# mttga/purejaxql

Hardware: NVIDIA H100
Metric: MinAtar-Breakout env steps/sec @4096 envs x128 seeds (higher is better)
Workload: dtype f32

## Files before the change

include/pqn_b200.h:

```cpp
#ifndef PQN_B200_H
#define PQN_B200_H

#include <stdint.h>

#ifdef __cplusplus
extern "C" {
#endif

#define PQN_OK 0
#define PQN_E_INVALID (-1)
#define PQN_E_CUDA (-2)
#define PQN_E_UNSUPPORTED (-3)

#define PQN_ENV_BREAKOUT 0
#define PQN_ENV_ASTERIX 1
#define PQN_ENV_SPACE_INVADERS 2
#define PQN_ENV_FREEWAY 3
#define PQN_ENV_SEAQUEST 4
#define PQN_ENV_CARTPOLE 16
#define PQN_ENV_ACROBOT 17
#define PQN_ENV_MOUNTAIN_CAR 18
#define PQN_ENV_MEMORY_CHAIN 32
#define PQN_ENV_CATCH 33
#define PQN_ENV_DEEP_SEA 34
// ... 99 lines not shown

int pqn_net_layout(const pqn_net_desc_t* desc_host, pqn_net_layout_t* out_host);
int pqn_net_dense_layer(const pqn_net_desc_t* desc_host, int32_t layer, int64_t* offsets_host);
int64_t pqn_net_stats_floats(const pqn_net_desc_t* desc_host);
int64_t pqn_net_workspace_bytes(const pqn_net_desc_t* desc_host, int32_t S, int64_t rows);

int pqn_net_init(const pqn_net_desc_t* desc_host, const uint32_t* keys, float* params, int32_t S, void* stream);

int pqn_qnet_forward(const pqn_net_desc_t* desc_host, const float* params, const float* batch_stats, const void* obs,
                     const int32_t* gather, int64_t obs_rows_per_seed, float* q, int32_t S, int64_t rows,
                     void* workspace, void* stream);

int pqn_qnet_loss_grad(const pqn_net_desc_t* desc_host, const float* params, float* batch_stats, const void* obs,
                       const int32_t* gather, int64_t obs_rows_per_seed, const int32_t* action,
                       const float* target, int64_t tr_rows_per_seed, float* grads, float* loss_sum,
                       float* qsa_sum, float* bn_sums, int32_t S, int64_t rows, void* workspace, void* stream);

int pqn_rnn_step(const pqn_net_desc_t* desc_host, const float* params, float* hs, const float* obs,
                 int64_t obs_rows_per_seed, const uint8_t* last_done, const int32_t* last_action, float* q, int32_t S,
                 int32_t E, void* workspace, void* stream);
int pqn_rnn_loss_grad(const pqn_net_desc_t* desc_host, const float* params, const float* hs0, const float* obs,
                      const uint8_t* last_done, const int32_t* last_action, const int32_t* action, const float* reward,
                      const uint8_t* done, float* grads, float* loss_sum, float* qsa_sum, int32_t S, int32_t T, int32_t B,
                      float gamma, float lambda, void* workspace, void* stream);
int pqn_rnn_step_stats(const pqn_net_desc_t* desc_host, const float* params, const float* batch_stats, float* hs,
                       const float* obs, int64_t obs_rows_per_seed, const uint8_t* last_done, const int32_t* last_action,
                       float* q, int32_t S, int32_t E, void* workspace, void* stream);
int pqn_rnn_loss_grad_stats(const pqn_net_desc_t* desc_host, const float* params, float* batch_stats, const float* hs0,
                            const float* obs, const uint8_t* last_done, const int32_t* last_action,
                            const int32_t* action, const float* reward, const uint8_t* done, float* grads,
                            float* loss_sum, float* qsa_sum, int32_t S, int32_t T, int32_t B, float gamma, float lambda,
                            void* workspace, void* stream);

int pqn_radam_clip_step(float* params, const float* grads, float* mu, float* nu, const float* sched,
                        int32_t* step_counter, float* gnorm_scratch , int32_t S, int64_t P,
                        float max_norm, float b1, float b2, float eps, void* stream);

int pqn_bn_stats_update(float* batch_stats, float* bn_sums, int32_t S, int32_t F, int64_t stats_seed_stride,
                        float count, float momentum, void* stream);

int pqn_set_tensor_core_path(int on);
int pqn_set_conv_mma_path(int on);

int pqn_tc_split_lo(const float* x, float* lo, int64_t n, void* stream);
int pqn_tc_gemm_test(const float* a, const float* a_lo, const float* b, const float* b_lo, float* d, int32_t S,
                     int32_t M, int32_t N, int32_t K, int a_mn, int b_mn, int split3, void* stream);

int pqn_tc_split16(const float* x, void* hi, void* lo, int64_t n, float scale, void* stream);
int pqn_tc_gemm16_test(const void* a_hi, const void* a_lo, const void* b_hi, const void* b_lo, float* d, int32_t S,
                       int32_t M, int32_t N, int32_t K, int a_mn, int b_mn, float out_scale, void* stream);
int pqn_tc_dgrad16_test(const void* a_hi, const void* a_lo, const void* b_hi, const void* b_lo, const float* mask,
                        const uint32_t* relu_bits, float* d, int32_t S, int32_t M, int32_t N, int32_t K, int epi,
                        float out_scale, void* stream);

#ifdef __cplusplus
}
#endif
#endif
```

purejaxql_b200/_lib.py:

```python
from __future__ import annotations

import ctypes
import os
from ctypes import POINTER, Structure, c_char_p, c_double, c_float, c_int, c_int32, c_int64, c_longlong, c_void_p

HERE = os.path.dirname(os.path.abspath(__file__))
LIB_PATH = os.path.join(HERE, "libpqn_b200.so")


class EnvInfo(Structure):
    _fields_ = [("state_words", c_int32), ("obs_dim", c_int32), ("obs_shape", c_int32 * 3),
                ("num_actions", c_int32), ("max_steps", c_int32), ("binary_obs", c_int32),
                ("packed_obs_words", c_int32)]


class EnvParams(Structure):
    _fields_ = [("max_steps", c_int32), ("memory_length", c_int32)]


class NetDesc(Structure):
    _fields_ = [("kind", c_int32), ("in_c", c_int32), ("hidden", c_int32), ("layers", c_int32),
                ("num_actions", c_int32), ("norm_type", c_int32), ("norm_input", c_int32)]


# ... 25 lines not shown
    "pqn_threefry2x32": (c_int, [c_void_p, c_void_p, c_void_p, c_int64, c_void_p]),
    "pqn_rng_bits": (c_int, [c_void_p, c_int64, c_int64, c_void_p, c_int, c_void_p]),
    "pqn_random_normal": (c_int, [c_void_p, c_void_p, c_int64, c_int, c_void_p]),
    "pqn_normal_from_bits": (c_int, [c_void_p, c_void_p, c_int64, c_void_p]),
    "pqn_set_permutation_bucket_log2": (c_int, [c_int]),
    "pqn_permutation_workspace_bytes": (c_int64, [c_int64, c_int]),
    "pqn_permutation": (c_int, [c_void_p, c_int64, c_int, c_int, c_void_p, c_int64, c_void_p, c_void_p]),
    "pqn_env_reset": (c_int, [c_int, c_void_p, c_void_p, c_void_p, c_int64, c_int, c_int, c_void_p]),
    "pqn_env_reset_params": (c_int, [c_int, c_void_p, c_void_p, c_void_p, c_int64, POINTER(EnvParams), c_int, c_void_p]),
    "pqn_env_step": (c_int, [c_int, c_void_p, c_void_p, c_void_p, c_void_p, c_void_p, c_void_p, c_void_p,
                             c_void_p, c_void_p, c_void_p, c_int64, c_int, c_int, c_void_p]),
    "pqn_env_obs_packed": (c_int, [c_int, c_void_p, c_void_p, c_int64, c_void_p]),
    "pqn_env_obs": (c_int, [c_int, c_void_p, c_void_p, c_int64, c_void_p]),
    "pqn_eps_greedy": (c_int, [c_void_p, c_void_p, c_void_p, c_void_p, c_int64, c_int32, c_int, c_void_p]),
    "pqn_rollout_act_step": (c_int, [c_int, c_void_p, c_void_p, c_void_p, c_void_p, c_void_p, c_int64, c_void_p,
                                     c_void_p, c_void_p, c_void_p, c_int64, c_void_p, c_int, c_int32, c_int32,
                                     c_int32, c_int32, c_int, c_float, c_int, c_void_p]),
    "pqn_rollout_keys": (c_int, [c_void_p, c_void_p, c_int32, c_int32, c_int, c_void_p]),
    "pqn_qlambda": (c_int, [c_void_p, c_void_p, c_void_p, c_void_p, c_void_p, c_int32, c_int32, c_int32, c_int32,
                            c_float, c_float, c_void_p]),
    "pqn_net_layout": (c_int, [POINTER(NetDesc), POINTER(NetLayout)]),
    "pqn_net_dense_layer": (c_int, [POINTER(NetDesc), c_int32, POINTER(c_int64)]),
    "pqn_net_stats_floats": (c_int64, [POINTER(NetDesc)]),
    "pqn_net_workspace_bytes": (c_int64, [POINTER(NetDesc), c_int32, c_int64]),
    "pqn_net_init": (c_int, [POINTER(NetDesc), c_void_p, c_void_p, c_int32, c_void_p]),
    "pqn_qnet_forward": (c_int, [POINTER(NetDesc), c_void_p, c_void_p, c_void_p, c_void_p, c_int64, c_void_p, c_int32,
                                 c_int64, c_void_p, c_void_p]),
    "pqn_qnet_loss_grad": (c_int, [POINTER(NetDesc), c_void_p, c_void_p, c_void_p, c_void_p, c_int64, c_void_p,
                                   c_void_p, c_int64, c_void_p, c_void_p, c_void_p, c_void_p, c_int32, c_int64,
                                   c_void_p, c_void_p]),
    "pqn_rnn_step": (c_int, [POINTER(NetDesc), c_void_p, c_void_p, c_void_p, c_int64, c_void_p, c_void_p, c_void_p,
                             c_int32, c_int32, c_void_p, c_void_p]),
    "pqn_rnn_loss_grad": (c_int, [POINTER(NetDesc), c_void_p, c_void_p, c_void_p, c_void_p, c_void_p, c_void_p, c_void_p,
                                  c_void_p, c_void_p, c_void_p, c_void_p, c_int32, c_int32, c_int32, c_float, c_float,
                                  c_void_p, c_void_p]),
    "pqn_rnn_step_stats": (c_int, [POINTER(NetDesc), c_void_p, c_void_p, c_void_p, c_void_p, c_int64, c_void_p, c_void_p,
                                   c_void_p, c_int32, c_int32, c_void_p, c_void_p]),
    "pqn_rnn_loss_grad_stats": (c_int, [POINTER(NetDesc), c_void_p, c_void_p, c_void_p, c_void_p, c_void_p, c_void_p,
                                        c_void_p, c_void_p, c_void_p, c_void_p, c_void_p, c_void_p, c_int32, c_int32,
                                        c_int32, c_float, c_float, c_void_p, c_void_p]),
    "pqn_radam_clip_step": (c_int, [c_void_p, c_void_p, c_void_p, c_void_p, c_void_p, c_void_p, c_void_p, c_int32,
                                    c_int64, c_float, c_float, c_float, c_float, c_void_p]),
    "pqn_bn_stats_update": (c_int, [c_void_p, c_void_p, c_int32, c_int32, c_int64, c_float, c_float, c_void_p]),
    "pqn_set_tensor_core_path": (c_int, [c_int]),
    "pqn_set_conv_mma_path": (c_int, [c_int]),
    "pqn_tc_split_lo": (c_int, [c_void_p, c_void_p, c_int64, c_void_p]),
    "pqn_tc_split16": (c_int, [c_void_p, c_void_p, c_void_p, c_int64, c_float, c_void_p]),
    "pqn_tc_gemm_test": (c_int, [c_void_p, c_void_p, c_void_p, c_void_p, c_void_p, c_int32, c_int32, c_int32,
                                 c_int32, c_int, c_int, c_int, c_void_p]),
    "pqn_tc_gemm16_test": (c_int, [c_void_p, c_void_p, c_void_p, c_void_p, c_void_p, c_int32, c_int32, c_int32,
                                   c_int32, c_int, c_int, c_float, c_void_p]),
    "pqn_tc_dgrad16_test": (c_int, [c_void_p, c_void_p, c_void_p, c_void_p, c_void_p, c_void_p, c_void_p, c_int32,
                                    c_int32, c_int32, c_int32, c_int, c_float, c_void_p]),
}

EXPORTS = tuple(_SIGS)
_lib = None


def lib():
    global _lib
    if _lib is None:
        if not os.path.exists(LIB_PATH):
            raise PqnError(
                f"{LIB_PATH} is not built. Run `python -m purejaxql_b200.build` (needs nvcc). "
                "purejaxql_b200 has no CPU fallback.")
        l = ctypes.CDLL(LIB_PATH)
        for name, (res, args) in _SIGS.items():
            fn = getattr(l, name)
            fn.restype = res
            fn.argtypes = args
        _lib = l
    return _lib


def check(rc: int, what: str = ""):
    if rc != 0:
        msg = lib().pqn_last_error().decode("utf-8", "replace")
        raise PqnError(f"{what or 'libpqn_b200'} failed (rc={rc}): {msg}")


def p(t):
    if t is None:
        return None
    if not t.is_cuda:
        raise PqnError("libpqn_b200 takes CUDA tensors only (no CPU fallback); got a CPU tensor")
    if not t.is_contiguous():
        raise PqnError("libpqn_b200 takes contiguous tensors")
    return c_void_p(t.data_ptr())


def raw(t):
    if t is None:
        return None
    if not t.is_cuda:
        raise PqnError("libpqn_b200 takes CUDA tensors only (no CPU fallback); got a CPU tensor")
    return c_void_p(t.data_ptr())


def stream_ptr():
    import torch
    return c_void_p(torch.cuda.current_stream().cuda_stream)


def profile_read(reset=True):
    l = lib()
# ... 6 lines not shown
```

purejaxql_b200/csrc/pqn_tc.cu:

```cuda
#include <cuda.h>
#include <cuda_runtime.h>
#include <stdint.h>

#include "../../include/pqn_b200.h"
#include "api_common.h"
#include "tc_common.cuh"

namespace pqn {
namespace tc {

constexpr int STG_LD = 36;

__device__ __forceinline__ void store_chunk_coalesced(float* stage, const float (&vals)[32], int lane, float* dst,
                                                      int64_t ld, int m_base, int M) {
#pragma unroll
  for (int j = 0; j < 8; ++j)
    *reinterpret_cast<float4*>(stage + lane * STG_LD + 4 * j) =
        make_float4(vals[4 * j], vals[4 * j + 1], vals[4 * j + 2], vals[4 * j + 3]);
  __syncwarp();
  const int r_in = lane >> 3, c4 = lane & 7;
#pragma unroll
  for (int it = 0; it < 8; ++it) {
    const int r = it * 4 + r_in;
    if (m_base + r < M)
// ... 46 lines not shown
  const float rstd = 1.0f / sqrtf(var + 1e-6f);
  const int64_t grow = (int64_t)seed * ep.rows + m;
  if constexpr (EPI == EPI_LN_TRAIN) {
    float* hbase = ep.H + ((int64_t)seed * ep.rows + m_base) * 128;
    float* xbase = ep.XHAT + ((int64_t)seed * ep.rows + m_base) * 128;
#pragma unroll
    for (int c = 0; c < 4; ++c) {
      float xh[32], h[32];
#pragma unroll
      for (int j4 = 0; j4 < 8; ++j4) {
        const float4 s4 = *reinterpret_cast<const float4*>(sp + SP_SC + c * 32 + 4 * j4);
        const float4 b4 = *reinterpret_cast<const float4*>(sp + SP_BI + c * 32 + 4 * j4);
        const float ss[4] = {s4.x, s4.y, s4.z, s4.w}, bb[4] = {b4.x, b4.y, b4.z, b4.w};
#pragma unroll
        for (int e = 0; e < 4; ++e) {
          const int j = 4 * j4 + e;
          xh[j] = (acc[c * 32 + j] - mean) * rstd;
          h[j] = fmaxf(xh[j] * ss[e] + bb[e], 0.f);
        }
      }
      store_chunk_coalesced(stage, h, lane, hbase + c * 32, 128, m_base, M);
      store_chunk_coalesced(stage, xh, lane, xbase + c * 32, 128, m_base, M);
    }
    if (row_ok) ep.RSTD[grow] = rstd;
  } else {
    float q[PQN_TC_MAX_A];
#pragma unroll
    for (int a = 0; a < PQN_TC_MAX_A; ++a) q[a] = 0.f;
#pragma unroll
    for (int j4 = 0; j4 < 32; ++j4) {
      const float4 s4 = *reinterpret_cast<const float4*>(sp + SP_SC + 4 * j4);
      const float4 b4 = *reinterpret_cast<const float4*>(sp + SP_BI + 4 * j4);
      float h[4];
      h[0] = fmaxf((acc[4 * j4 + 0] - mean) * rstd * s4.x + b4.x, 0.f);
      h[1] = fmaxf((acc[4 * j4 + 1] - mean) * rstd * s4.y + b4.y, 0.f);
      h[2] = fmaxf((acc[4 * j4 + 2] - mean) * rstd * s4.z + b4.z, 0.f);
      h[3] = fmaxf((acc[4 * j4 + 3] - mean) * rstd * s4.w + b4.w, 0.f);
#pragma unroll
      for (int a = 0; a < PQN_TC_MAX_A; ++a)
        if (a < ep.A) {
          const float4 w4 = *reinterpret_cast<const float4*>(sp + SP_HW + a * 128 + 4 * j4);
          q[a] = fmaf(h[0], w4.x, q[a]); q[a] = fmaf(h[1], w4.y, q[a]);
          q[a] = fmaf(h[2], w4.z, q[a]); q[a] = fmaf(h[3], w4.w, q[a]);
        }
    }
    if (row_ok) {
#pragma unroll
      for (int a = 0; a < PQN_TC_MAX_A; ++a)
        if (a < ep.A) ep.Q[grow * ep.A + a] = q[a] + sp[SP_HB + a];
    }
  }
}

template <int MN>
__device__ __forceinline__ float lds_tf32(const uint8_t* tile, int r, int k) {
  const int off = MN ? ((r >> 5) * 4096 + k * 128 + ((((r & 31) >> 2) ^ (k & 7)) << 4) + ((r & 3) << 2))
                     : (r * 128 + (((k >> 2) ^ (r & 7)) << 4) + ((k & 3) << 2));
  return *reinterpret_cast<const float*>(tile + off);
}
__device__ __forceinline__ uint32_t tf32_trunc_bits(float x) { return __float_as_uint(x) & 0xFFFFE000u; }
__device__ __forceinline__ void mma_tf32_16x8x8(float (&d)[4], const uint32_t (&a)[4], uint32_t b0, uint32_t b1) {
  asm volatile(
      "mma.sync.aligned.m16n8k8.row.col.f32.tf32.tf32.f32 {%0,%1,%2,%3}, {%4,%5,%6,%7}, {%8,%9}, {%0,%1,%2,%3};"
      : "+f"(d[0]), "+f"(d[1]), "+f"(d[2]), "+f"(d[3])
      : "r"(a[0]), "r"(a[1]), "r"(a[2]), "r"(a[3]), "r"(b0), "r"(b1));
}

template <int A_MN, int B_MN>
__device__ __forceinline__ void tf32_tile(const uint8_t* smem_al, float* tile_s, uint64_t* full, uint64_t* empty,
                                          int& stage, uint32_t& phase, int kbn, int split3, float osc, int warp,
                                          int lane) {
  const int g = lane >> 2, tq = lane & 3;
  const int wr = (warp & 3) * 32, wc = (warp >> 2) * 64;
  float mainacc[2][8][4], corr[2][8][4];
#pragma unroll
  for (int mi = 0; mi < 2; ++mi)
#pragma unroll
    for (int ni = 0; ni < 8; ++ni)
#pragma unroll
      for (int e = 0; e < 4; ++e) { mainacc[mi][ni][e] = 0.f; corr[mi][ni][e] = 0.f; }
  for (int kb = 0; kb < kbn; ++kb) {
    mbar_wait(&full[stage], phase);
    const uint8_t* sb = smem_al + stage * TC_STAGE_BYTES;
    if (kb % TC_PROMOTE == 0) {
#pragma unroll
      for (int mi = 0; mi < 2; ++mi)
#pragma unroll
        for (int ni = 0; ni < 8; ++ni)
#pragma unroll
          for (int e = 0; e < 4; ++e) mainacc[mi][ni][e] = 0.f;
    }
#pragma unroll
    for (int ks = 0; ks < TC_BK / 8; ++ks) {
      const int k = ks * 8 + tq;
      uint32_t ahi[2][4], alo[2][4];
#pragma unroll
      for (int mi = 0; mi < 2; ++mi) {
        const int r0 = wr + mi * 16 + g;
        const int rr[4] = {r0, r0 + 8, r0, r0 + 8}, kk[4] = {k, k, k + 4, k + 4};
#pragma unroll
        for (int e = 0; e < 4; ++e) {
          const float x = lds_tf32<A_MN>(sb + TC_A_HI, rr[e], kk[e]);
          ahi[mi][e] = tf32_trunc_bits(x);
          const float lo = split3 == 1 ? lds_tf32<A_MN>(sb + TC_A_LO, rr[e], kk[e]) : x - __uint_as_float(ahi[mi][e]);
          alo[mi][e] = tf32_trunc_bits(lo);
        }
      }
#pragma unroll
      for (int ni = 0; ni < 8; ++ni) {
        const int n = wc + ni * 8 + g;
        const uint32_t bh0 = tf32_trunc_bits(lds_tf32<B_MN>(sb + TC_B_HI, n, k));
        const uint32_t bh1 = tf32_trunc_bits(lds_tf32<B_MN>(sb + TC_B_HI, n, k + 4));
        if (split3) {
          const uint32_t bl0 = tf32_trunc_bits(lds_tf32<B_MN>(sb + TC_B_LO, n, k));
          const uint32_t bl1 = tf32_trunc_bits(lds_tf32<B_MN>(sb + TC_B_LO, n, k + 4));
#pragma unroll
          for (int mi = 0; mi < 2; ++mi) {
            mma_tf32_16x8x8(corr[mi][ni], alo[mi], bh0, bh1);
            mma_tf32_16x8x8(corr[mi][ni], ahi[mi], bl0, bl1);
          }
        }
#pragma unroll
        for (int mi = 0; mi < 2; ++mi) mma_tf32_16x8x8(mainacc[mi][ni], ahi[mi], bh0, bh1);
      }
    }
    __syncwarp();
    if (lane == 0) mbar_arrive(&empty[stage]);
    if (++stage == TC_STAGES) { stage = 0; phase ^= 1u; }
    if ((kb + 1) % TC_PROMOTE == 0 || kb == kbn - 1) {
      const bool first = kb < TC_PROMOTE;
#pragma unroll
      for (int mi = 0; mi < 2; ++mi)
#pragma unroll
        for (int ni = 0; ni < 8; ++ni)
#pragma unroll
          for (int h = 0; h < 2; ++h) {
            float2* p = reinterpret_cast<float2*>(tile_s + (wr + mi * 16 + g + 8 * h) * TC_ACC_LD + wc + ni * 8 + 2 * tq);
            const float2 v = make_float2(mainacc[mi][ni][2 * h], mainacc[mi][ni][2 * h + 1]);
            if (first) *p = v;
            else { const float2 o = *p; *p = make_float2(o.x + v.x, o.y + v.y); }
          }
    }
  }
#pragma unroll
  for (int mi = 0; mi < 2; ++mi)
#pragma unroll
    for (int ni = 0; ni < 8; ++ni)
#pragma unroll
      for (int h = 0; h < 2; ++h) {
        float2* p = reinterpret_cast<float2*>(tile_s + (wr + mi * 16 + g + 8 * h) * TC_ACC_LD + wc + ni * 8 + 2 * tq);
        float2 o = kbn > 0 ? *p : make_float2(0.f, 0.f);
        o.x += corr[mi][ni][2 * h];
        o.y += corr[mi][ni][2 * h + 1];
        *p = make_float2(o.x * osc, o.y * osc);
      }
}

template <int EPI, bool F16>
__host__ __device__ constexpr bool tma_store_epilogue() { return F16 && (EPI == EPI_RELU_MASK || EPI == EPI_RELU_BITS); }

__device__ __forceinline__ void wg_bar_sync(int wg) { asm volatile("bar.sync %0, 128;" ::"r"(3 + wg) : "memory"); }

template <int A_MN, int B_MN, int EPI, bool F16 = true>
__global__ void __launch_bounds__(TC_THREADS, 1)
    tc_gemm_kernel(const __grid_constant__ CUtensorMap tm_a_hi, const __grid_constant__ CUtensorMap tm_a_lo,
                   const __grid_constant__ CUtensorMap tm_b_hi, const __grid_constant__ CUtensorMap tm_b_lo,
                   const __grid_constant__ CUtensorMap tm_out, const GemmShape gs, const EpiParams ep) {
  constexpr bool TMA_EPI = tma_store_epilogue<EPI, F16>();
  extern __shared__ __align__(1024) uint8_t smem_raw[];
  const uint32_t smem_base = (smem_u32(smem_raw) + 1023u) & ~1023u;
  uint8_t* smem_al = smem_raw + (smem_base - smem_u32(smem_raw));
  float* tile_s = reinterpret_cast<float*>(smem_al + TC_STAGES * TC_STAGE_BYTES);
  float* sp_all = tile_s + 128 * TC_ACC_LD;
  uint64_t* full = reinterpret_cast<uint64_t*>(sp_all + TC_SP_FLOATS);
  uint64_t* empty = full + TC_STAGES;

  const int warp = threadIdx.x >> 5, lane = threadIdx.x & 31;

  if (warp == 8 && lane == 0) {
    prefetch_tmap(&tm_a_hi); prefetch_tmap(&tm_a_lo); prefetch_tmap(&tm_b_hi); prefetch_tmap(&tm_b_lo);
    if (TMA_EPI) prefetch_tmap(&tm_out);
    for (int i = 0; i < TC_STAGES; ++i) { mbar_init(&full[i], 1); mbar_init(&empty[i], TC_CONSUMERS / 32); }
    fence_barrier_init();
  }
  __syncthreads();

  const int ksplit = gs.k_split > 1 ? gs.k_split : 1;
  const int kb_per = (gs.k_blocks + ksplit - 1) / ksplit;
  const int tiles_per_seed = gs.m_tiles * gs.n_tiles * ksplit;
  const int num_tiles = tiles_per_seed * gs.S;
  auto decode = [&](int tile, int& seed, int& m0, int& n0, int& kb0, int& kbn) {
    seed = tile / tiles_per_seed;
    const int rem = tile - seed * tiles_per_seed;
    const int ks = rem % ksplit, mn = rem / ksplit;
    m0 = (mn / gs.n_tiles) * 128; n0 = (mn % gs.n_tiles) * 128;
    kb0 = ks * kb_per;
    kbn = min(kb_per, gs.k_blocks - kb0);
    if (kbn < 0) kbn = 0;
    return ks;
  };

  constexpr int BKE = F16 ? TC_BK16 : TC_BK;
  constexpr int MNB = F16 ? 2 : 4;
  constexpr int MNB_ELEMS = F16 ? 64 : 32, MNB_BYTES = F16 ? 8192 : 4096;
  const bool a_lo_tma = F16 || gs.split3 == 1, b_lo_tma = F16 || gs.split3 != 0;
  if (warp == 8) {
    if (lane == 0) {
      int stage = 0;
      uint32_t phase = 0;
      for (int tile = blockIdx.x; tile < num_tiles; tile += gridDim.x) {
        int seed, m0, n0, kb0, kbn;
        decode(tile, seed, m0, n0, kb0, kbn);
        for (int kb = kb0; kb < kb0 + kbn; ++kb) {
          mbar_wait(&empty[stage], phase ^ 1u);
          const uint32_t sb = smem_base + stage * TC_STAGE_BYTES;
          mbar_expect_tx(&full[stage], (2 + (a_lo_tma ? 1 : 0) + (b_lo_tma ? 1 : 0)) * TC_TILE_BYTES);
          const int k0 = kb * BKE;
          if (A_MN) {
#pragma unroll
            for (int j = 0; j < MNB; ++j) {
              tma_load_3d(sb + TC_A_HI + j * MNB_BYTES, &tm_a_hi, &full[stage], m0 + MNB_ELEMS * j, k0, seed);
              if (a_lo_tma) tma_load_3d(sb + TC_A_LO + j * MNB_BYTES, &tm_a_lo, &full[stage], m0 + MNB_ELEMS * j, k0, seed);
            }
          } else {
            tma_load_3d(sb + TC_A_HI, &tm_a_hi, &full[stage], k0, m0, seed);
            if (a_lo_tma) tma_load_3d(sb + TC_A_LO, &tm_a_lo, &full[stage], k0, m0, seed);
          }
          if (B_MN) {
#pragma unroll
            for (int j = 0; j < MNB; ++j) {
              tma_load_3d(sb + TC_B_HI + j * MNB_BYTES, &tm_b_hi, &full[stage], n0 + MNB_ELEMS * j, k0, seed);
              if (b_lo_tma) tma_load_3d(sb + TC_B_LO + j * MNB_BYTES, &tm_b_lo, &full[stage], n0 + MNB_ELEMS * j, k0, seed);
            }
          } else {
            tma_load_3d(sb + TC_B_HI, &tm_b_hi, &full[stage], k0, n0, seed);
            if (b_lo_tma) tma_load_3d(sb + TC_B_LO, &tm_b_lo, &full[stage], k0, n0, seed);
          }
          if (++stage == TC_STAGES) { stage = 0; phase ^= 1u; }
        }
      }
    }
    return;
  }

  const int t = threadIdx.x;
  const int wg = t >> 7;
  const uint32_t a_off = wg * 8192;
  const int fr = 64 * wg + 16 * ((t & 127) >> 5) + (lane >> 2), fc = 2 * (lane & 3);
  const int et = t & 127;
  uint8_t* out_stage = reinterpret_cast<uint8_t*>(tile_s) + wg * TC_OUT_STAGE_WG;
  int stage = 0;
  uint32_t phase = 0;
  for (int tile = blockIdx.x; tile < num_tiles; tile += gridDim.x) {
    int seed, m0, n0, kb0, kbn;
    const int ks_idx = decode(tile, seed, m0, n0, kb0, kbn);
    uint32_t rbits[2][4];
    if constexpr (TMA_EPI) {
      if constexpr (EPI == EPI_RELU_BITS) {
#pragma unroll
        for (int h = 0; h < 2; ++h) {
          const int m = m0 + fr + 8 * h;
          const uint4 w = m < gs.M ? __ldg(reinterpret_cast<const uint4*>(
                                         ep.relu_bits + ((int64_t)seed * ep.rows + m) * (ep.ld_out >> 5) + (n0 >> 5)))
                                   : make_uint4(0u, 0u, 0u, 0u);
          rbits[h][0] = w.x; rbits[h][1] = w.y; rbits[h][2] = w.z; rbits[h][3] = w.w;
        }
      } else {
        const int m = m0 + 64 * wg + (et >> 1);
        const float* p = ep.mask + (int64_t)seed * ep.out_seed_stride + (int64_t)m * ep.ld_out + n0 + 64 * (et & 1);
        if (m < gs.M) {
          asm volatile("prefetch.global.L2 [%0];" ::"l"(p));
          asm volatile("prefetch.global.L2 [%0];" ::"l"(p + 32));
        }
      }
      if (kbn > TC_PROMOTE) {
        if (et == 0) bulk_wait_read_all();
        wg_bar_sync(wg);
      }
    } else {
      consumer_bar_sync();
    }
    if constexpr (!F16) {
      tf32_tile<A_MN, B_MN>(smem_al, tile_s, full, empty, stage, phase, kbn, gs.split3,
                            ep.out_scale != 0.f ? ep.out_scale : 1.0f, warp, lane);
    } else {
    float mainacc[64], corr[64];
#pragma unroll
    for (int i = 0; i < 64; ++i) { mainacc[i] = 0.f; corr[i] = 0.f; }
    for (int kb = 0; kb < kbn; ++kb) {
      mbar_wait(&full[stage], phase);
      const uint32_t sb = smem_base + stage * TC_STAGE_BYTES;
      const uint32_t first_corr = kb == 0 ? 0u : 1u, first_main = kb % TC_PROMOTE == 0 ? 0u : 1u;
      fence_operands(mainacc); fence_operands(corr);
      wgmma_fence();
#pragma unroll
      for (int ks = 0; ks < 4; ++ks) {
        const uint64_t a_hi = make_gdesc16<A_MN>(sb + TC_A_HI + a_off, ks), a_lo = make_gdesc16<A_MN>(sb + TC_A_LO + a_off, ks);
        const uint64_t b_hi = make_gdesc16<B_MN>(sb + TC_B_HI, ks), b_lo = make_gdesc16<B_MN>(sb + TC_B_LO, ks);
        wgmma_f16_m64n128<A_MN, B_MN>(corr, a_lo, b_hi, ks == 0 ? first_corr : 1u);
        wgmma_f16_m64n128<A_MN, B_MN>(corr, a_hi, b_lo, 1u);
        wgmma_f16_m64n128<A_MN, B_MN>(mainacc, a_hi, b_hi, ks == 0 ? first_main : 1u);
      }
      wgmma_commit();
      wgmma_wait<0>();
      fence_operands(mainacc); fence_operands(corr);
      __syncwarp();
      if (lane == 0) mbar_arrive(&empty[stage]);
      if (++stage == TC_STAGES) { stage = 0; phase ^= 1u; }
      const bool promote = TMA_EPI ? (kb + 1) % TC_PROMOTE == 0 && kb != kbn - 1
                                   : (kb + 1) % TC_PROMOTE == 0 || kb == kbn - 1;
      if (promote) {
        const bool first = kb < TC_PROMOTE;
#pragma unroll
        for (int j = 0; j < 16; ++j)
#pragma unroll
          for (int h = 0; h < 2; ++h) {
            float2* p = reinterpret_cast<float2*>(tile_s + (fr + 8 * h) * TC_ACC_LD + 8 * j + fc);
            const float2 v = make_float2(mainacc[4 * j + 2 * h], mainacc[4 * j + 2 * h + 1]);
            if (first) *p = v;
            else { const float2 o = *p; *p = make_float2(o.x + v.x, o.y + v.y); }
          }
      }
    }
    if constexpr (TMA_EPI) {
      const float osc = ep.out_scale != 0.f ? ep.out_scale : 1.0f;
      const float* mrow = ep.mask + (int64_t)seed * ep.out_seed_stride + n0;
#pragma unroll
      for (int j = 0; j < 16; ++j)
#pragma unroll
        for (int h = 0; h < 2; ++h) {
          const int i = 4 * j + 2 * h;
          float2 o = make_float2(mainacc[i], mainacc[i + 1]);
          if (kbn > TC_PROMOTE) {
            const float2 p = *reinterpret_cast<const float2*>(tile_s + (fr + 8 * h) * TC_ACC_LD + 8 * j + fc);
            o = make_float2(p.x + o.x, p.y + o.y);
          }
          mainacc[i] = fmaf(corr[i], TC_LO_INV, o.x) * osc;
          mainacc[i + 1] = fmaf(corr[i + 1], TC_LO_INV, o.y) * osc;
        }
#pragma unroll
      for (int j = 0; j < 16; ++j)
#pragma unroll
        for (int h = 0; h < 2; ++h) {
          float& x = mainacc[4 * j + 2 * h];
          float& y = mainacc[4 * j + 2 * h + 1];
          if constexpr (EPI == EPI_RELU_BITS) {
            const uint32_t b = rbits[h][j >> 2] >> (8 * (j & 3) + fc);
            x = (b & 1u) ? x : 0.f; y = (b & 2u) ? y : 0.f;
          } else {
            const int m = m0 + fr + 8 * h;
            if (m < gs.M) {
              const float2 mk = *reinterpret_cast<const float2*>(mrow + (int64_t)m * ep.ld_out + 8 * j + fc);
              x = mk.x > 0.f ? x : 0.f; y = mk.y > 0.f ? y : 0.f;
            }
          }
        }
      if (et == 0) bulk_wait_read_all();
      wg_bar_sync(wg);
      const int rl = fr - 64 * wg;
#pragma unroll
      for (int j = 0; j < 16; ++j)
#pragma unroll
        for (int h = 0; h < 2; ++h) {
          const int chunk = 2 * (j & 3) + (fc >> 2);
          const int off = (j >> 2) * TC_OUT_BOX_BYTES + (rl + 8 * h) * 128 + ((chunk ^ (lane >> 2)) << 4) + (fc & 3) * 4;
          *reinterpret_cast<float2*>(out_stage + off) = make_float2(mainacc[4 * j + 2 * h], mainacc[4 * j + 2 * h + 1]);
        }
      fence_proxy_async_smem();
      wg_bar_sync(wg);
      if (et == 0) {
#pragma unroll
        for (int b = 0; b < 4; ++b)
          tma_store_3d(&tm_out, smem_u32(out_stage + b * TC_OUT_BOX_BYTES), n0 + 32 * b, m0 + 64 * wg, seed);
        bulk_commit();
      }
      continue;
    }
    {
      const float osc = ep.out_scale != 0.f ? ep.out_scale : 1.0f;
#pragma unroll
      for (int j = 0; j < 16; ++j)
#pragma unroll
        for (int h = 0; h < 2; ++h) {
          float2* p = reinterpret_cast<float2*>(tile_s + (fr + 8 * h) * TC_ACC_LD + 8 * j + fc);
          float2 o = kbn > 0 ? *p : make_float2(0.f, 0.f);
          if (kbn > 0) {
            o.x = fmaf(corr[4 * j + 2 * h], TC_LO_INV, o.x);
            o.y = fmaf(corr[4 * j + 2 * h + 1], TC_LO_INV, o.y);
          }
          *p = make_float2(o.x * osc, o.y * osc);
        }
    }
// ... 181 lines not shown

int pqn_tc_split16(const float* x, void* hi, void* lo, int64_t n, float scale, void* stream) {
  if (!x || !hi || !lo || n < 0 || (n & 3)) return set_error(PQN_E_INVALID, "pqn_tc_split16: bad argument (n %% 4 == 0)");
  if (n == 0) return PQN_OK;
  {
    LaunchScope _ls(K_TC_SPLIT, (cudaStream_t)stream);
    split16_kernel<<<(unsigned)((n / 4 + 255) / 256), 256, 0, (cudaStream_t)stream>>>(x, (__half*)hi, (__half*)lo, n / 4,
                                                                                       scale);
  }
  return check_launch("pqn_tc_split16");
}

int pqn_tc_gemm16_test(const void* a_hi, const void* a_lo, const void* b_hi, const void* b_lo, float* d, int32_t S,
                       int32_t M, int32_t N, int32_t K, int a_mn, int b_mn, float out_scale, void* stream) {
  if (!a_hi || !a_lo || !b_hi || !b_lo || !d || S <= 0 || M <= 0 || N <= 0 || K <= 0 || (N % 128) || (K % 8) || (M % 8))
    return set_error(PQN_E_INVALID, "pqn_tc_gemm16_test: bad argument");
  CUtensorMap t[4];
  int rc;
  const void* ap[2] = {a_hi, a_lo};
  const void* bp[2] = {b_hi, b_lo};
  for (int i = 0; i < 2; ++i) {
    if (a_mn) { if ((rc = make_tmap16(&t[i], ap[i], M, K, S, M, (uint64_t)M * K, 64))) return rc; }
    else { if ((rc = make_tmap16(&t[i], ap[i], K, M, S, K, (uint64_t)M * K, 128))) return rc; }
    if (b_mn) { if ((rc = make_tmap16(&t[2 + i], bp[i], N, K, S, N, (uint64_t)N * K, 64))) return rc; }
    else { if ((rc = make_tmap16(&t[2 + i], bp[i], K, N, S, K, (uint64_t)N * K, 128))) return rc; }
  }
  GemmShape gs = {};
  gs.S = S; gs.M = M; gs.m_tiles = (M + 127) / 128; gs.n_tiles = N / 128; gs.k_blocks = (K + TC_BK16 - 1) / TC_BK16;
  EpiParams ep = {};
  ep.out = d; ep.ld_out = N; ep.out_seed_stride = (int64_t)M * N; ep.out_scale = out_scale;
  return launch_gemm16(a_mn, b_mn, EPI_STORE, t, gs, ep, (cudaStream_t)stream);
}

int pqn_tc_dgrad16_test(const void* a_hi, const void* a_lo, const void* b_hi, const void* b_lo, const float* mask,
                        const uint32_t* relu_bits, float* d, int32_t S, int32_t M, int32_t N, int32_t K, int epi,
                        float out_scale, void* stream) {
  if (!a_hi || !a_lo || !b_hi || !b_lo || !d || S <= 0 || M <= 0 || N <= 0 || K <= 0 || (N % 128) || (K % 8) ||
      (M % 8) || !(epi == EPI_STORE || epi == EPI_RELU_MASK || epi == EPI_RELU_BITS) ||
      (epi == EPI_RELU_MASK && !mask) || (epi == EPI_RELU_BITS && !relu_bits))
    return set_error(PQN_E_INVALID, "pqn_tc_dgrad16_test: bad argument");
  CUtensorMap t[4];
  int rc;
  const void* p[4] = {a_hi, a_lo, b_hi, b_lo};
  for (int i = 0; i < 2; ++i) {
    if ((rc = make_tmap16(&t[i], p[i], K, M, S, K, (uint64_t)M * K, 128))) return rc;
    if ((rc = make_tmap16(&t[2 + i], p[2 + i], K, N, S, K, (uint64_t)N * K, 128))) return rc;
  }
  GemmShape gs = {};
  gs.S = S; gs.M = M; gs.m_tiles = (M + 127) / 128; gs.n_tiles = N / 128; gs.k_blocks = (K + TC_BK16 - 1) / TC_BK16;
  EpiParams ep = {};
  ep.out = d; ep.mask = mask; ep.relu_bits = relu_bits; ep.rows = M;
  ep.ld_out = N; ep.out_seed_stride = (int64_t)M * N; ep.out_scale = out_scale;
  return launch_gemm16(0, 0, epi, t, gs, ep, (cudaStream_t)stream);
}

int pqn_tc_gemm_test(const float* a, const float* a_lo, const float* b, const float* b_lo, float* d, int32_t S,
                     int32_t M, int32_t N, int32_t K, int a_mn, int b_mn, int split3, void* stream) {
  if (!a || !b || !d || S <= 0 || M <= 0 || N <= 0 || K <= 0 || (N % 128) || split3 < 0 || split3 > 2 ||
      (split3 && !b_lo) || (split3 == 1 && !a_lo))
    return set_error(PQN_E_INVALID, "pqn_tc_gemm_test: bad argument");
  CUtensorMap t[4];
  int rc;
  const float* al = split3 == 1 ? a_lo : a;
  const float* bl = split3 ? b_lo : b;
  const float* ap[2] = {a, al};
  const float* bp[2] = {b, bl};
  for (int i = 0; i < 2; ++i) {
    if (a_mn) { if ((rc = make_tmap(&t[i], ap[i], M, K, S, M, (uint64_t)M * K, 32))) return rc; }
    else { if ((rc = make_tmap(&t[i], ap[i], K, M, S, K, (uint64_t)M * K, 128))) return rc; }
    if (b_mn) { if ((rc = make_tmap(&t[2 + i], bp[i], N, K, S, N, (uint64_t)N * K, 32))) return rc; }
    else { if ((rc = make_tmap(&t[2 + i], bp[i], K, N, S, K, (uint64_t)N * K, 128))) return rc; }
  }
  GemmShape gs = {};
  gs.S = S; gs.M = M; gs.m_tiles = (M + 127) / 128; gs.n_tiles = N / 128; gs.k_blocks = (K + TC_BK - 1) / TC_BK;
  gs.split3 = split3;
  EpiParams ep = {};
  ep.out = d; ep.ld_out = N; ep.out_seed_stride = (int64_t)M * N;
  return launch_gemm(a_mn, b_mn, EPI_STORE, t, gs, ep, (cudaStream_t)stream);
}

}
```

purejaxql_b200/csrc/tc_common.cuh:

```cuda
#pragma once
#include <cuda.h>
#include <cuda_fp16.h>
#include <stdint.h>

namespace pqn {
namespace tc {

constexpr int TC_CONSUMERS = 256;
constexpr int TC_THREADS = TC_CONSUMERS + 32;
constexpr int TC_BK16 = 64;
constexpr int TC_BK = 32;
constexpr int TC_STAGES = 2;
constexpr int TC_PROMOTE = 4;
constexpr int TC_TILE_BYTES = 128 * TC_BK16 * 2;
constexpr float TC_LO_SCALE = 2048.0f, TC_LO_INV = 1.0f / 2048.0f;
constexpr int TC_A_HI = 0, TC_A_LO = TC_TILE_BYTES, TC_B_HI = 2 * TC_TILE_BYTES, TC_B_LO = 3 * TC_TILE_BYTES;
constexpr int TC_STAGE_BYTES = 4 * TC_TILE_BYTES;
constexpr int TC_ACC_LD = 132;
constexpr int TC_SP_FLOATS = 384 + 8 * 128 + 8;
constexpr int TC_SMEM_BYTES = TC_STAGES * TC_STAGE_BYTES + 128 * TC_ACC_LD * 4 + TC_SP_FLOATS * 4 + 256  +
                              1024 ;
constexpr int TC_OUT_BOX_BYTES = 64 * 32 * 4;
constexpr int TC_OUT_STAGE_WG = 34 * 1024;
static_assert(TC_OUT_STAGE_WG >= 64 * TC_ACC_LD * 4 && TC_OUT_STAGE_WG + 4 * TC_OUT_BOX_BYTES <= 128 * TC_ACC_LD * 4,
              "each warpgroup's output staging lies within its own 64 rows of the fp32 tile, 1024-byte aligned");
#define PQN_TC_MAX_A 8

enum Epilogue : int { EPI_STORE = 0, EPI_LN_TRAIN = 1, EPI_LN_HEAD = 2, EPI_RELU_MASK = 3, EPI_RELU_BITS = 4 };

struct GemmShape {
  int S;
  int M;
  int m_tiles, n_tiles, k_blocks;
  int split3;
  int k_split;
};

struct EpiParams {
  int64_t split_stride;
  float out_scale;
  float* out;
  const float* mask;
  const uint32_t* relu_bits;
  int64_t ld_out, out_seed_stride;
  const float* params;
  int64_t P, off_b, off_scale, off_bias, off_hw, off_hb;
  int A, rows;
  float *H, *XHAT, *RSTD, *Q;
};

__device__ __forceinline__ uint32_t smem_u32(const void* p) { return (uint32_t)__cvta_generic_to_shared(p); }

__device__ __forceinline__ float tf32_lo(float x) {
  const float hi = __uint_as_float(__float_as_uint(x) & 0xFFFFE000u);
  return x - hi;
}

__device__ __forceinline__ void mbar_init(uint64_t* bar, int count) {
  asm volatile("mbarrier.init.shared::cta.b64 [%0], %1;" ::"r"(smem_u32(bar)), "r"(count) : "memory");
}
__device__ __forceinline__ void fence_barrier_init() { asm volatile("fence.mbarrier_init.release.cluster;" ::: "memory"); }
__device__ __forceinline__ void mbar_expect_tx(uint64_t* bar, uint32_t bytes) {
  asm volatile("mbarrier.arrive.expect_tx.shared::cta.b64 _, [%0], %1;" ::"r"(smem_u32(bar)), "r"(bytes) : "memory");
}
__device__ __forceinline__ void mbar_arrive(uint64_t* bar) {
  asm volatile("mbarrier.arrive.shared::cta.b64 _, [%0];" ::"r"(smem_u32(bar)) : "memory");
}
__device__ __forceinline__ void mbar_wait(uint64_t* bar, uint32_t parity) {
  const uint32_t addr = smem_u32(bar);
  uint32_t ok;
  do {
    asm volatile(
        "{\n\t.reg .pred p;\n\t"
        "mbarrier.try_wait.parity.shared::cta.b64 p, [%1], %2;\n\t"
        "selp.u32 %0, 1, 0, p;\n\t}"
        : "=r"(ok)
        : "r"(addr), "r"(parity)
        : "memory");
  } while (!ok);
}

__device__ __forceinline__ void prefetch_tmap(const CUtensorMap* tm) {
  asm volatile("prefetch.tensormap [%0];" ::"l"(reinterpret_cast<uint64_t>(tm)) : "memory");
}
__device__ __forceinline__ void tma_load_3d(uint32_t smem_dst, const CUtensorMap* tm, uint64_t* bar, int c0, int c1, int c2) {
  asm volatile(
      "cp.async.bulk.tensor.3d.shared::cluster.global.mbarrier::complete_tx::bytes [%0], [%1, {%3, %4, %5}], [%2];"
      ::"r"(smem_dst), "l"(reinterpret_cast<uint64_t>(tm)), "r"(smem_u32(bar)), "r"(c0), "r"(c1), "r"(c2)
      : "memory");
}
__device__ __forceinline__ void tma_store_3d(const CUtensorMap* tm, uint32_t smem_src, int c0, int c1, int c2) {
  asm volatile("cp.async.bulk.tensor.3d.global.shared::cta.bulk_group [%0, {%2, %3, %4}], [%1];"
               ::"l"(reinterpret_cast<uint64_t>(tm)), "r"(smem_src), "r"(c0), "r"(c1), "r"(c2)
               : "memory");
}
__device__ __forceinline__ void bulk_commit() { asm volatile("cp.async.bulk.commit_group;" ::: "memory"); }
__device__ __forceinline__ void bulk_wait_read_all() { asm volatile("cp.async.bulk.wait_group.read 0;" ::: "memory"); }
__device__ __forceinline__ void bulk_wait_all() { asm volatile("cp.async.bulk.wait_group 0;" ::: "memory"); }
__device__ __forceinline__ void fence_proxy_async_smem() { asm volatile("fence.proxy.async.shared::cta;" ::: "memory"); }

__device__ __forceinline__ void wgmma_fence() { asm volatile("wgmma.fence.sync.aligned;" ::: "memory"); }
__device__ __forceinline__ void wgmma_commit() { asm volatile("wgmma.commit_group.sync.aligned;" ::: "memory"); }
template <int N>
__device__ __forceinline__ void wgmma_wait() { asm volatile("wgmma.wait_group.sync.aligned %0;" ::"n"(N) : "memory"); }
__device__ __forceinline__ void fence_operands(float (&d)[64]) {
#pragma unroll
  for (int i = 0; i < 64; ++i) asm volatile("" : "+f"(d[i])::"memory");
}

template <int TA, int TB>
__device__ __forceinline__ void wgmma_f16_m64n128(float (&d)[64], uint64_t desc_a, uint64_t desc_b, uint32_t scale_d) {
  asm volatile(
      "{\n\t.reg .pred p;\n\t"
      "setp.ne.b32 p, %66, 0;\n\t"
      "wgmma.mma_async.sync.aligned.m64n128k16.f32.f16.f16 "
      "{%0, %1, %2, %3, %4, %5, %6, %7, %8, %9, %10, %11, %12, %13, %14, %15, %16, %17, %18, %19, %20, %21, %22, %23, "
      "%24, %25, %26, %27, %28, %29, %30, %31, %32, %33, %34, %35, %36, %37, %38, %39, %40, %41, %42, %43, %44, %45, "
      "%46, %47, %48, %49, %50, %51, %52, %53, %54, %55, %56, %57, %58, %59, %60, %61, %62, %63}, "
      "%64, %65, p, 1, 1, %67, %68;\n\t}"
      : "+f"(d[0]), "+f"(d[1]), "+f"(d[2]), "+f"(d[3]), "+f"(d[4]), "+f"(d[5]), "+f"(d[6]), "+f"(d[7]), "+f"(d[8]),
        "+f"(d[9]), "+f"(d[10]), "+f"(d[11]), "+f"(d[12]), "+f"(d[13]), "+f"(d[14]), "+f"(d[15]), "+f"(d[16]),
        "+f"(d[17]), "+f"(d[18]), "+f"(d[19]), "+f"(d[20]), "+f"(d[21]), "+f"(d[22]), "+f"(d[23]), "+f"(d[24]),
        "+f"(d[25]), "+f"(d[26]), "+f"(d[27]), "+f"(d[28]), "+f"(d[29]), "+f"(d[30]), "+f"(d[31]), "+f"(d[32]),
        "+f"(d[33]), "+f"(d[34]), "+f"(d[35]), "+f"(d[36]), "+f"(d[37]), "+f"(d[38]), "+f"(d[39]), "+f"(d[40]),
        "+f"(d[41]), "+f"(d[42]), "+f"(d[43]), "+f"(d[44]), "+f"(d[45]), "+f"(d[46]), "+f"(d[47]), "+f"(d[48]),
        "+f"(d[49]), "+f"(d[50]), "+f"(d[51]), "+f"(d[52]), "+f"(d[53]), "+f"(d[54]), "+f"(d[55]), "+f"(d[56]),
        "+f"(d[57]), "+f"(d[58]), "+f"(d[59]), "+f"(d[60]), "+f"(d[61]), "+f"(d[62]), "+f"(d[63])
      : "l"(desc_a), "l"(desc_b), "r"(scale_d), "n"(TA), "n"(TB));
}

template <int MN>
__device__ __forceinline__ uint64_t make_gdesc16(uint32_t tile_addr, int ks) {
  const uint32_t addr = MN ? tile_addr + ks * 2048 : tile_addr + ks * 32;
  const uint64_t lbo = MN ? (8192u >> 4) : 1u;
  const uint64_t sbo = 1024u >> 4;
  return (uint64_t)((addr >> 4) & 0x3FFFu) | (lbo << 16) | (sbo << 32) | (1ull << 62);
}

__device__ __forceinline__ void split16(float x, __half& hi, __half& lo) {
  x = fminf(fmaxf(x, -65000.0f), 65000.0f);
  hi = __float2half_rn(x);
  lo = __float2half_rn((x - __half2float(hi)) * TC_LO_SCALE);
}
template <bool SAT = true>
__device__ __forceinline__ void split16x2(float x0, float x1, __half2& hi, __half2& lo) {
  if (SAT) {
    x0 = fminf(fmaxf(x0, -65000.0f), 65000.0f);
    x1 = fminf(fmaxf(x1, -65000.0f), 65000.0f);
  }
  hi = __floats2half2_rn(x0, x1);
  const float2 hf = __half22float2(hi);
  lo = __floats2half2_rn((x0 - hf.x) * TC_LO_SCALE, (x1 - hf.y) * TC_LO_SCALE);
}
// ... 13 lines not shown
```

Measured before the change: 32.88 million.

## Add register-resident LayerNorm epilogue for f16 split wgmma dense forward

Adds a per-warpgroup LayerNorm (train and head) epilogue for the f16 hi/lo wgmma GEMM. Epilogue parameters are staged asynchronously with cp.async while the main loop runs, and row statistics are computed from register fragments through shared memory using warp shuffles. This replaces the shared consumer-barrier path for these epilogues and doubles the per-block parameter buffer. It is exposed through a new test entry point, so whether the benchmarked training path uses it is unclear.

Result: faster. 33.77 million, median of 6 (+2.7%).

```diff
diff --git a/include/pqn_b200.h b/include/pqn_b200.h
--- a/include/pqn_b200.h
+++ b/include/pqn_b200.h
@@ -175,6 +175,9 @@
 int pqn_tc_dgrad16_test(const void* a_hi, const void* a_lo, const void* b_hi, const void* b_lo, const float* mask,
                         const uint32_t* relu_bits, float* d, int32_t S, int32_t M, int32_t N, int32_t K, int epi,
                         float out_scale, void* stream);
+int pqn_tc_dense_fwd16_test(const void* h1_hi, const void* h1_lo, const void* w1_hi, const void* w1_lo,
+                            const float* params, float* h, float* xhat, float* rstd, float* q, int32_t S, int32_t M,
+                            int32_t K, int epi, int32_t A, void* stream);
 
 #ifdef __cplusplus
 }
diff --git a/purejaxql_b200/_lib.py b/purejaxql_b200/_lib.py
--- a/purejaxql_b200/_lib.py
+++ b/purejaxql_b200/_lib.py
@@ -101,6 +101,8 @@
                                    c_int32, c_int, c_int, c_float, c_void_p]),
     "pqn_tc_dgrad16_test": (c_int, [c_void_p, c_void_p, c_void_p, c_void_p, c_void_p, c_void_p, c_void_p, c_int32,
                                     c_int32, c_int32, c_int32, c_int, c_float, c_void_p]),
+    "pqn_tc_dense_fwd16_test": (c_int, [c_void_p, c_void_p, c_void_p, c_void_p, c_void_p, c_void_p, c_void_p,
+                                        c_void_p, c_void_p, c_int32, c_int32, c_int32, c_int, c_int32, c_void_p]),
 }
 
 EXPORTS = tuple(_SIGS)
diff --git a/purejaxql_b200/csrc/pqn_tc.cu b/purejaxql_b200/csrc/pqn_tc.cu
--- a/purejaxql_b200/csrc/pqn_tc.cu
+++ b/purejaxql_b200/csrc/pqn_tc.cu
@@ -122,6 +122,120 @@
   }
 }
 
+template <int EPI>
+__device__ __forceinline__ void stage_epi_params_async(const EpiParams& ep, float* sp, int seed, int et ) {
+  const float* __restrict__ prm = ep.params + (int64_t)seed * ep.P;
+  cp_async4(sp + SP_B + et, prm + ep.off_b + et);
+  cp_async4(sp + SP_SC + et, prm + ep.off_scale + et);
+  cp_async4(sp + SP_BI + et, prm + ep.off_bias + et);
+  if constexpr (EPI == EPI_LN_HEAD) {
+    for (int a = 0; a < ep.A; ++a) cp_async4(sp + SP_HW + a * 128 + et, prm + ep.off_hw + (int64_t)et * ep.A + a);
+    if (et < ep.A) cp_async4(sp + SP_HB + et, prm + ep.off_hb + et);
+  }
+  cp_async_commit();
+}
+
+template <int EPI>
+__device__ __forceinline__ void epilogue_ln_frag(const EpiParams& ep, float (&v)[64], float* tile_s, const float* sp,
+                                                 int seed, int m0, int fr, int fc, int lane, int M) {
+  const int q = lane & 3, qbase = lane & ~3;
+  const float* row = tile_s + (fr + 8 * (q >> 1)) * TC_ACC_LD;
+#pragma unroll
+  for (int j = 0; j < 16; ++j) {
+    const float2 b = *reinterpret_cast<const float2*>(sp + SP_B + 8 * j + fc);
+#pragma unroll
+    for (int h = 0; h < 2; ++h) {
+      v[4 * j + 2 * h] += b.x; v[4 * j + 2 * h + 1] += b.y;
+      *reinterpret_cast<float2*>(tile_s + (fr + 8 * h) * TC_ACC_LD + 8 * j + fc) =
+          make_float2(v[4 * j + 2 * h], v[4 * j + 2 * h + 1]);
+    }
+  }
+  __syncwarp();
+  float s = 0.f;
+  const bool sq = q & 1;
+#pragma unroll 4
+  for (int j4 = 0; j4 < 32; ++j4) {
+    const float4 x = *reinterpret_cast<const float4*>(row + 4 * j4);
+    s = fmaf(x.x, sq ? x.x : 1.f, s); s = fmaf(x.y, sq ? x.y : 1.f, s);
+    s = fmaf(x.z, sq ? x.z : 1.f, s); s = fmaf(x.w, sq ? x.w : 1.f, s);
+  }
+  float mean[2], rstd[2];
+#pragma unroll
+  for (int h = 0; h < 2; ++h) {
+    const float s1 = __shfl_sync(0xffffffffu, s, qbase + 2 * h), s2 = __shfl_sync(0xffffffffu, s, qbase + 2 * h + 1);
+    mean[h] = s1 * (1.0f / 128.f);
+    const float var = fmaxf(s2 * (1.0f / 128.f) - mean[h] * mean[h], 0.f);
+    rstd[h] = 1.0f / sqrtf(var + 1e-6f);
+  }
+#pragma unroll
+  for (int j = 0; j < 16; ++j)
+#pragma unroll
+    for (int h = 0; h < 2; ++h) {
+      const float2 x = *reinterpret_cast<const float2*>(tile_s + (fr + 8 * h) * TC_ACC_LD + 8 * j + fc);
+      v[4 * j + 2 * h] = x.x; v[4 * j + 2 * h + 1] = x.y;
+    }
+  if constexpr (EPI == EPI_LN_TRAIN) {
+#pragma unroll
+    for (int h = 0; h < 2; ++h) {
+      const int m = m0 + fr + 8 * h;
+      if (m >= M) continue;
+      const int64_t grow = (int64_t)seed * ep.rows + m;
+      float* hrow = ep.H + grow * 128 + fc;
+      float* xrow = ep.XHAT + grow * 128 + fc;
+#pragma unroll
+      for (int j = 0; j < 16; ++j) {
+        const float2 s = *reinterpret_cast<const float2*>(sp + SP_SC + 8 * j + fc);
+        const float2 bi = *reinterpret_cast<const float2*>(sp + SP_BI + 8 * j + fc);
+        const float xh0 = (v[4 * j + 2 * h] - mean[h]) * rstd[h], xh1 = (v[4 * j + 2 * h + 1] - mean[h]) * rstd[h];
+        *reinterpret_cast<float2*>(hrow + 8 * j) = make_float2(fmaxf(xh0 * s.x + bi.x, 0.f), fmaxf(xh1 * s.y + bi.y, 0.f));
+        *reinterpret_cast<float2*>(xrow + 8 * j) = make_float2(xh0, xh1);
+      }
+      if (q == 0) ep.RSTD[grow] = rstd[h];
+    }
+  } else {
+    __syncwarp();
+#pragma unroll
+    for (int j = 0; j < 16; ++j) {
+      const float2 s = *reinterpret_cast<const float2*>(sp + SP_SC + 8 * j + fc);
+      const float2 bi = *reinterpret_cast<const float2*>(sp + SP_BI + 8 * j + fc);
+#pragma unroll
+      for (int h = 0; h < 2; ++h) {
+        const float h0 = fmaxf((v[4 * j + 2 * h] - mean[h]) * rstd[h] * s.x + bi.x, 0.f);
+        const float h1 = fmaxf((v[4 * j + 2 * h + 1] - mean[h]) * rstd[h] * s.y + bi.y, 0.f);
+        *reinterpret_cast<float2*>(tile_s + (fr + 8 * h) * TC_ACC_LD + 8 * j + fc) = make_float2(h0, h1);
+      }
+    }
+    __syncwarp();
+    constexpr int NA = PQN_TC_MAX_A / 2;
+    float qa[NA];
+#pragma unroll
+    for (int i = 0; i < NA; ++i) qa[i] = 0.f;
+#pragma unroll 4
+    for (int j4 = 0; j4 < 32; ++j4) {
+      const float4 hv = *reinterpret_cast<const float4*>(row + 4 * j4);
+#pragma unroll
+      for (int i = 0; i < NA; ++i) {
+        const int a = (q & 1) + 2 * i;
+        if (a < ep.A) {
+          const float4 w = *reinterpret_cast<const float4*>(sp + SP_HW + a * 128 + 4 * j4);
+          qa[i] = fmaf(hv.x, w.x, qa[i]); qa[i] = fmaf(hv.y, w.y, qa[i]);
+          qa[i] = fmaf(hv.z, w.z, qa[i]); qa[i] = fmaf(hv.w, w.w, qa[i]);
+        }
+      }
+    }
+    const int m = m0 + fr + 8 * (q >> 1);
+    if (m < M) {
+      const int64_t grow = (int64_t)seed * ep.rows + m;
+#pragma unroll
+      for (int i = 0; i < NA; ++i) {
+        const int a = (q & 1) + 2 * i;
+        if (a < ep.A) ep.Q[grow * ep.A + a] = qa[i] + sp[SP_HB + a];
+      }
+    }
+  }
+  __syncwarp();
+}
+
 template <int MN>
 __device__ __forceinline__ float lds_tf32(const uint8_t* tile, int r, int k) {
   const int off = MN ? ((r >> 5) * 4096 + k * 128 + ((((r & 31) >> 2) ^ (k & 7)) << 4) + ((r & 3) << 2))
@@ -228,6 +342,8 @@
 
 template <int EPI, bool F16>
 __host__ __device__ constexpr bool tma_store_epilogue() { return F16 && (EPI == EPI_RELU_MASK || EPI == EPI_RELU_BITS); }
+template <int EPI, bool F16>
+__host__ __device__ constexpr bool ln_reg_epilogue() { return F16 && (EPI == EPI_LN_TRAIN || EPI == EPI_LN_HEAD); }
 
 __device__ __forceinline__ void wg_bar_sync(int wg) { asm volatile("bar.sync %0, 128;" ::"r"(3 + wg) : "memory"); }
 
@@ -237,12 +353,14 @@
                    const __grid_constant__ CUtensorMap tm_b_hi, const __grid_constant__ CUtensorMap tm_b_lo,
                    const __grid_constant__ CUtensorMap tm_out, const GemmShape gs, const EpiParams ep) {
   constexpr bool TMA_EPI = tma_store_epilogue<EPI, F16>();
+  constexpr bool LN_REG = ln_reg_epilogue<EPI, F16>();
+  constexpr bool REG_EPI = TMA_EPI || LN_REG;
   extern __shared__ __align__(1024) uint8_t smem_raw[];
   const uint32_t smem_base = (smem_u32(smem_raw) + 1023u) & ~1023u;
   uint8_t* smem_al = smem_raw + (smem_base - smem_u32(smem_raw));
   float* tile_s = reinterpret_cast<float*>(smem_al + TC_STAGES * TC_STAGE_BYTES);
   float* sp_all = tile_s + 128 * TC_ACC_LD;
-  uint64_t* full = reinterpret_cast<uint64_t*>(sp_all + TC_SP_FLOATS);
+  uint64_t* full = reinterpret_cast<uint64_t*>(sp_all + 2 * TC_SP_FLOATS);
   uint64_t* empty = full + TC_STAGES;
 
   const int warp = threadIdx.x >> 5, lane = threadIdx.x & 31;
@@ -319,6 +437,7 @@
   const int fr = 64 * wg + 16 * ((t & 127) >> 5) + (lane >> 2), fc = 2 * (lane & 3);
   const int et = t & 127;
   uint8_t* out_stage = reinterpret_cast<uint8_t*>(tile_s) + wg * TC_OUT_STAGE_WG;
+  float* sp_wg = sp_all + wg * TC_SP_FLOATS;
   int stage = 0;
   uint32_t phase = 0;
   for (int tile = blockIdx.x; tile < num_tiles; tile += gridDim.x) {
@@ -347,6 +466,9 @@
         if (et == 0) bulk_wait_read_all();
         wg_bar_sync(wg);
       }
+    } else if constexpr (LN_REG) {
+      wg_bar_sync(wg);
+      stage_epi_params_async<EPI>(ep, sp_wg, seed, et);
     } else {
       consumer_bar_sync();
     }
@@ -377,7 +499,7 @@
       __syncwarp();
       if (lane == 0) mbar_arrive(&empty[stage]);
       if (++stage == TC_STAGES) { stage = 0; phase ^= 1u; }
-      const bool promote = TMA_EPI ? (kb + 1) % TC_PROMOTE == 0 && kb != kbn - 1
+      const bool promote = REG_EPI ? (kb + 1) % TC_PROMOTE == 0 && kb != kbn - 1
                                    : (kb + 1) % TC_PROMOTE == 0 || kb == kbn - 1;
       if (promote) {
         const bool first = kb < TC_PROMOTE;
@@ -392,9 +514,8 @@
           }
       }
     }
-    if constexpr (TMA_EPI) {
+    if constexpr (REG_EPI) {
       const float osc = ep.out_scale != 0.f ? ep.out_scale : 1.0f;
-      const float* mrow = ep.mask + (int64_t)seed * ep.out_seed_stride + n0;
 #pragma unroll
       for (int j = 0; j < 16; ++j)
 #pragma unroll
@@ -408,6 +529,13 @@
           mainacc[i] = fmaf(corr[i], TC_LO_INV, o.x) * osc;
           mainacc[i + 1] = fmaf(corr[i + 1], TC_LO_INV, o.y) * osc;
         }
+      if constexpr (LN_REG) {
+        cp_async_wait_all();
+        wg_bar_sync(wg);
+        epilogue_ln_frag<EPI>(ep, mainacc, tile_s, sp_wg, seed, m0, fr, fc, lane, gs.M);
+        continue;
+      }
+      const float* mrow = ep.mask + (int64_t)seed * ep.out_seed_stride + n0;
 #pragma unroll
       for (int j = 0; j < 16; ++j)
 #pragma unroll
@@ -695,6 +823,32 @@
   ep.out = d; ep.mask = mask; ep.relu_bits = relu_bits; ep.rows = M;
   ep.ld_out = N; ep.out_seed_stride = (int64_t)M * N; ep.out_scale = out_scale;
   return launch_gemm16(0, 0, epi, t, gs, ep, (cudaStream_t)stream);
+}
+
+int pqn_tc_dense_fwd16_test(const void* h1_hi, const void* h1_lo, const void* w1_hi, const void* w1_lo,
+                            const float* params, float* h, float* xhat, float* rstd, float* q, int32_t S, int32_t M,
+                            int32_t K, int epi, int32_t A, void* stream) {
+  if (!h1_hi || !h1_lo || !w1_hi || !w1_lo || !params || S <= 0 || M <= 0 || K <= 0 || (K % 8) || (M % 8) ||
+      !(epi == EPI_LN_TRAIN || epi == EPI_LN_HEAD) || (epi == EPI_LN_TRAIN && (!h || !xhat || !rstd)) ||
+      (epi == EPI_LN_HEAD && (!q || A < 1 || A > PQN_TC_MAX_A)))
+    return set_error(PQN_E_INVALID, "pqn_tc_dense_fwd16_test: bad argument");
+  CUtensorMap t[4];
+  int rc;
+  const void* hp[2] = {h1_hi, h1_lo};
+  const void* wp[2] = {w1_hi, w1_lo};
+  for (int i = 0; i < 2; ++i) {
+    if ((rc = make_tmap16(&t[i], hp[i], K, M, S, K, (uint64_t)M * K, 128))) return rc;
+    if ((rc = make_tmap16(&t[2 + i], wp[i], 128, K, S, 128, (uint64_t)K * 128, 64))) return rc;
+  }
+  GemmShape gs = {};
+  gs.S = S; gs.M = M; gs.m_tiles = (M + 127) / 128; gs.n_tiles = 1; gs.k_blocks = (K + TC_BK16 - 1) / TC_BK16;
+  EpiParams ep = {};
+  const int a = epi == EPI_LN_HEAD ? A : 1;
+  ep.params = params; ep.P = 384 + 129 * a;
+  ep.off_b = 0; ep.off_scale = 128; ep.off_bias = 256; ep.off_hw = 384; ep.off_hb = 384 + 128 * a;
+  ep.A = a; ep.rows = M;
+  ep.H = h; ep.XHAT = xhat; ep.RSTD = rstd; ep.Q = q;
+  return launch_gemm16(0, 1, epi, t, gs, ep, (cudaStream_t)stream);
 }
 
 int pqn_tc_gemm_test(const float* a, const float* a_lo, const float* b, const float* b_lo, float* d, int32_t S,
diff --git a/purejaxql_b200/csrc/tc_common.cuh b/purejaxql_b200/csrc/tc_common.cuh
--- a/purejaxql_b200/csrc/tc_common.cuh
+++ b/purejaxql_b200/csrc/tc_common.cuh
@@ -18,8 +18,8 @@
 constexpr int TC_STAGE_BYTES = 4 * TC_TILE_BYTES;
 constexpr int TC_ACC_LD = 132;
 constexpr int TC_SP_FLOATS = 384 + 8 * 128 + 8;
-constexpr int TC_SMEM_BYTES = TC_STAGES * TC_STAGE_BYTES + 128 * TC_ACC_LD * 4 + TC_SP_FLOATS * 4 + 256  +
-                              1024 ;
+constexpr int TC_SMEM_BYTES = TC_STAGES * TC_STAGE_BYTES + 128 * TC_ACC_LD * 4 + 2 * TC_SP_FLOATS * 4 +
+                              256  + 1024 ;
 constexpr int TC_OUT_BOX_BYTES = 64 * 32 * 4;
 constexpr int TC_OUT_STAGE_WG = 34 * 1024;
 static_assert(TC_OUT_STAGE_WG >= 64 * TC_ACC_LD * 4 && TC_OUT_STAGE_WG + 4 * TC_OUT_BOX_BYTES <= 128 * TC_ACC_LD * 4,
@@ -99,6 +99,12 @@
 __device__ __forceinline__ void bulk_wait_all() { asm volatile("cp.async.bulk.wait_group 0;" ::: "memory"); }
 __device__ __forceinline__ void fence_proxy_async_smem() { asm volatile("fence.proxy.async.shared::cta;" ::: "memory"); }
 
+__device__ __forceinline__ void cp_async4(void* smem_dst, const void* gsrc) {
+  asm volatile("cp.async.ca.shared.global [%0], [%1], 4;" ::"r"(smem_u32(smem_dst)), "l"(gsrc) : "memory");
+}
+__device__ __forceinline__ void cp_async_commit() { asm volatile("cp.async.commit_group;" ::: "memory"); }
+__device__ __forceinline__ void cp_async_wait_all() { asm volatile("cp.async.wait_group 0;" ::: "memory"); }
+
 __device__ __forceinline__ void wgmma_fence() { asm volatile("wgmma.fence.sync.aligned;" ::: "memory"); }
 __device__ __forceinline__ void wgmma_commit() { asm volatile("wgmma.commit_group.sync.aligned;" ::: "memory"); }
 template <int N>
```
